# tsilva/gymnasium-solver

Measured on AMD Instinct MI355X. Metric: env steps/sec (rollout+PPO update), CartPole n_envs=4096, 1/2/4/8 MI355X, higher is better.
Workload: dtype f32; 1 GPU; CartPole-v1:ppo C2 (rollout 4096 envs x 32 steps + 20-epoch PPO update, B=256); n_envs_per_gpu=4096, n_steps=32, batch_size=256, n_epochs=20, policy=MLP 4-256-256-{2,1}, parallelism=single, graph=True, same_device=False, dp_mode=local, track_stats=False

## Files before the change

gymnasium-solver_amd/build_lib.py:

```python
from __future__ import annotations

import os
import subprocess
import sys
from concurrent.futures import ThreadPoolExecutor

HERE = os.path.dirname(os.path.abspath(__file__))
CSRC = os.path.join(HERE, "csrc")
BUILD = os.path.join(HERE, "build")
LIB = os.path.join(HERE, "gsamd", "libgsamd.so")
HIPCC = os.environ.get("HIPCC", "/opt/rocm/bin/hipcc")
ARCH = "gfx950"

EXTRA = {"gs_gae.hip": ["-ffp-contract=off"], "gs_mlp.hip": ["-ffp-contract=off"], "gs_atari.hip": ["-ffp-contract=off"],
         "gs_cartpole.hip": ["-ffp-contract=off"]}


def _sources():
    return sorted(f for f in os.listdir(CSRC) if f.endswith((".hip", ".cpp")))


def _obj(src):
    return os.path.join(BUILD, src + ".o")


def _source_hashes(csrc=None):
    sys.path.insert(0, os.path.join(HERE, "gsamd"))
    try:
        import buildinfo
    finally:
# ... 6 lines not shown
def _compile(src, build_dir=None, defines=(), csrc=None, hashes=None):
    csrc = csrc or CSRC
    path = os.path.join(csrc, src)
    obj = os.path.join(build_dir, src + ".o") if build_dir else _obj(src)
    deps = [path, os.path.join(HERE, "..", "include", "gsamd.h")] + [
        os.path.join(csrc, h) for h in os.listdir(csrc) if h.endswith(".h")]
    hdefs = []
    if src == "gs_abi.cpp" and hashes:
        hdefs = [f'-DGS_SRC_HASH_{k}="{v}"' for k, v in sorted(hashes.items())]
        stamp = obj + ".hash"
        if not os.path.exists(stamp) or open(stamp).read() != " ".join(hdefs):
            if os.path.exists(obj):
                os.remove(obj)
            with open(stamp, "w") as f:
                f.write(" ".join(hdefs))
    if os.path.exists(obj) and os.path.getmtime(obj) >= max(os.path.getmtime(d) for d in deps):
        return None
    cmd = [HIPCC, "-O3", "-std=c++17", "-fPIC", "-Wall", "-Wno-unused-function", "-c", path, "-o", obj]
    if src.endswith(".hip"):
        cmd[1:1] = [f"--offload-arch={ARCH}", "-x", "hip"]
    cmd += EXTRA.get(src, []) + [f"-D{d}" for d in defines] + hdefs
    r = subprocess.run(cmd, capture_output=True, text=True)
    if r.returncode != 0:
        raise RuntimeError(f"compile failed: {' '.join(cmd)}\n{r.stdout}\n{r.stderr}")
    return src


def build(verbose: bool = False, jobs: int = 8) -> str:
    os.makedirs(BUILD, exist_ok=True)
    srcs = _sources()
    hashes = _source_hashes()
    with ThreadPoolExecutor(max_workers=min(jobs, len(srcs))) as ex:
        done = [s for s in ex.map(lambda s: _compile(s, hashes=hashes), srcs) if s]
    objs = [_obj(s) for s in srcs]
    if done or not os.path.exists(LIB) or os.path.getmtime(LIB) < max(os.path.getmtime(o) for o in objs):
        cmd = [HIPCC, f"--offload-arch={ARCH}", "-shared", "-fPIC", "-o", LIB] + objs + [
            "-L/opt/rocm/lib", "-lrccl", "-Wl,-rpath,/opt/rocm/lib"]
        r = subprocess.run(cmd, capture_output=True, text=True)
        if r.returncode != 0:
# ... 39 lines not shown
```

gymnasium-solver_amd/csrc/gs_common.h:

```cpp
#pragma once
#include <hip/hip_runtime.h>
#include <stdint.h>
#include <stdio.h>
#include <string>
#include <type_traits>

#include "../../include/gsamd.h"

typedef float f32x4 __attribute__((ext_vector_type(4)));
typedef __bf16 bf16x8 __attribute__((ext_vector_type(8)));

namespace gs {

#ifdef GS_STAMPS
extern __device__ unsigned long long g_stamp_acc[8][16];
extern __device__ unsigned long long g_stamp_cnt[8];
#define GS_STAMP_BEGIN_IF(k, cond)                                                 \
    unsigned long long _st_t[17];                                                  \
    int _st_n = 0;                                                                 \
    const bool _st_on = (cond) && threadIdx.x == 0;                                \
    const int _st_k = (k);                                                         \
    if (_st_on) _st_t[0] = __builtin_amdgcn_s_memtime();
#define GS_STAMP_BEGIN(k) GS_STAMP_BEGIN_IF(k, blockIdx.x == 0 && blockIdx.y == 0)
#define GS_STAMP(i)                                                                \
    if (_st_on) _st_t[(i) + 1] = __builtin_amdgcn_s_memtime();                     \
    _st_n = (i) + 1;
#define GS_STAMP_END(i)                                                            \
    GS_STAMP(i)                                                                    \
    if (_st_on) {                                                                  \
        for (int _j = 0; _j < _st_n; ++_j)                                         \
            atomicAdd(&g_stamp_acc[_st_k][_j], _st_t[_j + 1] - _st_t[_j]);         \
        atomicAdd(&g_stamp_cnt[_st_k], 1ull);                                      \
    }
#else
#define GS_STAMP_BEGIN(k)
#define GS_STAMP_BEGIN_IF(k, cond)
#define GS_STAMP(i)
#define GS_STAMP_END(i)
#endif

void set_error(const char *fmt, ...);
int hip_fail(hipError_t e, const char *what, const char *file, int line);

#define GS_HIP(call)                                                         \
    do {                                                                     \
        hipError_t _e = (call);                                              \
        if (_e != hipSuccess) return gs::hip_fail(_e, #call, __FILE__, __LINE__); \
    } while (0)

#define GS_REQUIRE(cond, ...)                    \
// ... 315 lines not shown
```

gymnasium-solver_amd/csrc/gs_mlp.hip:

```cpp
#include <float.h>

#include <mutex>
#include <unordered_map>

#include "gs_common.h"
#include "gs_xgmi_dev.h"
#include "gs_synth_env.h"

namespace gs {

#ifdef GS_STAMPS
__device__ unsigned long long g_stamp_acc[8][16];
__device__ unsigned long long g_stamp_cnt[8];
#endif
#if defined(GS_STAMPS) || defined(GS_SPANS)
constexpr int kSpanK = 2048, kSpanWG = 288;
__device__ unsigned g_span[2][kSpanK][kSpanWG][9];
__device__ __forceinline__ int span_wg() { return (int)(blockIdx.x + blockIdx.y * gridDim.x); }
__device__ __forceinline__ void span_start(int kern, int64_t k, unsigned long long t0)
{
    if (threadIdx.x == 0 && k >= 0 && k < kSpanK && span_wg() < kSpanWG) g_span[kern][k][span_wg()][0] = (unsigned)t0;
}
__device__ __forceinline__ void span_end(int kern, int64_t k)
{
// ... 168 lines not shown

template <int AMAX, int AEX>
__device__ __forceinline__ void gather_head_row(const float *__restrict__ zpart, const float *__restrict__ P,
                                                const Layout &L, int64_t r, float (&z)[AMAX + 1]);
template <int AMAX>
__device__ __forceinline__ void loss_row(const float (&z)[AMAX + 1], int A, int act, float olp, float ov, float adv,
                                         float ret, const LossArgs &la, float invB, float *__restrict__ dzr,
                                         double (&acc)[14]);

#ifndef GS_FWD_ADAM_NT
#define GS_FWD_ADAM_NT 512
#endif
constexpr int kFwdAdamThreads = GS_FWD_ADAM_NT;
static_assert(kFwdAdamThreads == 256 || kFwdAdamThreads == 512, "lagged forward: 256 or 512 threads");

template <class S, bool FUSED, bool ADAM = false, bool STATS = false>
__global__ __launch_bounds__(ADAM ? kFwdAdamThreads : 256) void k_fwd_hidden(
    const float *__restrict__ P, Layout Lrt, const float *__restrict__ obs, const int32_t *__restrict__ idx, int T,
    int N, int rows, float *__restrict__ x_out, float *__restrict__ h1_out, float *__restrict__ h2_out,
    float *__restrict__ zpart, float *__restrict__ obs_copy, const int32_t *__restrict__ stop, RowGather rg,
    FusedFwd ff, LossArgs la, uint16_t *__restrict__ h2mask, AdamFwd af = AdamFwd{})
{
    GS_STAMP_BEGIN(0)
    GS_SPAN_T0
    if (stop && *stop) return;
    extern __shared__ float lds[];
    const Layout L = S::lay(Lrt);
    const int D = L.D, H1 = L.H1, H2 = L.H2, A1 = L.A + 1;
    const int cb = blockIdx.x, rb = blockIdx.y;
    const int r0 = rb * kTile;
    const int c0 = cb * kTile;
    const int tid = threadIdx.x, lane = tid & 63, wave = tid >> 6;
    constexpr int NT = ADAM ? kFwdAdamThreads : 256;
    const int ldh = H1 + 4;
    int *srcs = reinterpret_cast<int *>(lds);
    float *W1s = lds + 16;
    float *b1s = W1s + round4(H1 * D);
    float *W2s = b1s + round4(H1);
    float *b2s = W2s + kTile * ldh;
    float *whs = b2s + 16;
    float *xs = whs + round4(A1 * 16);
    float *h1s = xs + round4(kTile * D);
    float *red = h1s + kTile * ldh;
    float *h2s = red + 1024;

    if (rg.step_base && idx) idx += *rg.step_base * rows;
    const int64_t kstep = FUSED ? ff.k_local + (ff.step_base ? *ff.step_base : 0) : 0;
    if constexpr (ADAM) GS_SPAN_START(0, kstep)
    constexpr bool kStage0 = FUSED && S::H1c > 0 && (S::H1c * 4) % 4 == 0;
    constexpr int kW2v = S::H1c > 0 ? kTile * S::H1c / 4 / NT : 0;
    float4 w2r[kW2v > 0 ? kW2v : 1];
    static_assert(!ADAM || (kStage0 && kW2v > 0), "lagged Adam: compile-time fused shapes only");
    if constexpr (ADAM) {
        constexpr Layout Lc = S::lay(Layout{});
        constexpr int cD = Lc.D, cH1 = Lc.H1, cA1 = Lc.A + 1, n1 = cH1 * (cD + 1), k4n = cH1 / 4;
        constexpr int NQ = (n1 / 4 + 255) / 256, NRB = (S::Bc + S::RB - 1) / S::RB, NS = 2;
        static_assert(Lc.oW1 == 0 && Lc.oW2 == n1 && (cH1 * cD) % 4 == 0 && cH1 % 4 == 0, "W1|b1: one float4 region");
        static_assert(NRB >= 1 && NRB <= 8 && NQ <= 2 && n1 <= kTile * (cH1 + 4), "lagged-Adam register / LDS budget");
        const AdamArgs &aa = af.aa;
        const bool fold = af.part1 != nullptr;
        const int64_t kprev = kstep - 1 + af.force;
        const bool apply = kprev >= 0;
        const bool own1 = apply && cb == 0 && rb == 0, own2 = apply && rb == 0;
        const bool stW2[3] = {own2, own2, own2};
        const bool stW1[3] = {own1, own1, own1};
        const float4 z4 = make_float4(0.f, 0.f, 0.f, 0.f);
        auto ld4 = [](const float *base, int64_t q) {
            const f32x4 v = *(const __attribute__((address_space(1))) f32x4 *)(base + 4 * q);
            return make_float4(v[0], v[1], v[2], v[3]);
        };
        auto ld1 = [](const float *base, int64_t o) { return *(const __attribute__((address_space(1))) float *)(base + o); };
        constexpr int nq1 = n1 / 4;
        constexpr int NQP = (nq1 + NT - 1) / NT;
        const bool nrm = NT == 256 || tid < 256;
        float sl[NS];
#pragma unroll
        for (int j = 0; j < NS; ++j) sl[j] = ld1(af.sumsq, nrm ? min(tid + 256 * j, aa.n_slots - 1) : 0);
        float4 w1p[NQP], w1m[NQP], w1v[NQP], t[NQ][NRB];
        const float *tsrc = fold ? af.part1 : af.G;
        const int64_t tstride = fold ? (int64_t)n1 : 0;
        const int nrb_used = fold ? NRB : 1;
#pragma unroll
        for (int j = 0; j < NQ; ++j)
#pragma unroll
            for (int b = 0; b < NRB; ++b)
                t[j][b] = ld4(tsrc + (int64_t)b * tstride, nrm ? min(tid + 256 * j, nq1 - 1) : 0);
#pragma unroll
        for (int j = 0; j < NQP; ++j) {
            const int q = min(tid + NT * j, nq1 - 1);
            w1p[j] = ld4(P, q);
            w1m[j] = ld4(af.Min, q);
            w1v[j] = ld4(af.Vin, q);
// ... 433 lines not shown
    }
    const int ncbz = gridDim.x;
    for (int u = tid; u < kTile * A1; u += NT) {
        const int row = u / A1, a = u - row * A1;
        if (r0 + row >= rows) continue;
        float z = 0.0f;
#pragma unroll
        for (int c = 0; c < kTile; ++c) z = fmaf(h2s[row * 17 + c], whs[a * 16 + c], z);
        zpart[((int64_t)(r0 + row) * ncbz + cb) * A1 + a] = z;
    }
    if (!kEarly) store_x_h1(tid, NT);
    GS_STAMP_END(6)
    if constexpr (ADAM) GS_SPAN_END(0, kstep)
}

static int set_lds_limit(const void *fn, size_t bytes);
template <class F>
static int with_shape(const Layout &L, int64_t B, F &&f);

int launch_fwd_hidden(const float *params, const Layout &L, const float *obs, const int32_t *idx, int64_t T,
                      int64_t N, int64_t rows, float *x_out, float *h1_out, float *h2_out, float *zpart,
                      float *obs_copy, const int32_t *stop_flag, const RowGather *rg, hipStream_t s,
                      uint16_t *h2mask)
{
    const dim3 grid((unsigned)((L.H2 + kTile - 1) / kTile), (unsigned)((rows + kTile - 1) / kTile));
    RowGather g{};
    if (rg) g = *rg;
    return with_shape(L, 0, [&](auto sh) {
        using Sh = decltype(sh);
        int rc = set_lds_limit((const void *)k_fwd_hidden<Sh, false>, fwd_lds_bytes(L));
        if (rc) return rc;
        hipLaunchKernelGGL((k_fwd_hidden<Sh, false>), grid, dim3(256), fwd_lds_bytes(L), s, params, L, obs, idx,
                           (int)T, (int)N, (int)rows, x_out, h1_out, h2_out, zpart, obs_copy, stop_flag, g,
                           FusedFwd{}, LossArgs{}, h2_out ? h2mask : (uint16_t *)nullptr);
        GS_LAUNCH_CHECK("k_fwd_hidden");
        return GS_OK;
    });
}

struct HeadRow {
    float lse;
    float m2;
    float S;
};

template <int AMAX>
__device__ __forceinline__ HeadRow head_stats(const float (&z)[AMAX + 1], int A)
{
    float m = -INFINITY;
// ... 660 lines not shown
    }
}

__device__ __forceinline__ void store_metric_groups(const double *dscr, int n, int r0, int B, int64_t k,
                                                    double *__restrict__ mp)
{
    const int ng = n / kTile;
    if ((int)threadIdx.x < ng * kNumSums) {
        const int g = threadIdx.x / kNumSums, q = threadIdx.x - g * kNumSums;
        double t = 0.0;
        for (int i = 0; i < kTile; ++i) t += dscr[(g * kTile + i) * kNumSums + q];
        mp[(k * (B / kTile) + r0 / kTile + g) * kNumSums + q] = t;
    }
}

template <class S, bool FUSED>
__global__ __launch_bounds__(256) void k_bwd(const float *__restrict__ P, Layout Lrt, int Brt,
                                             const float *__restrict__ x, const float *__restrict__ h1,
                                             const float *__restrict__ h2, const float *__restrict__ dz,
                                             float *__restrict__ G, float *__restrict__ part1,
                                             float *__restrict__ sumsq, const int32_t *__restrict__ stop,
                                             const float *__restrict__ zpart, FusedFwd ff, LossArgs la,
                                             const uint16_t *__restrict__ h2mask, BwdXchg bx)
{
    GS_SPAN_T0
    if (stop && *stop) return;
    const bool xchg = bx.world > 1;
    const uint32_t xseq = xchg ? bx.seq[blockIdx.x] + 1u : 0u;
    const int64_t kstep = FUSED ? ff.k_local + (ff.step_base ? *ff.step_base : 0) : 0;
    if constexpr (FUSED) GS_SPAN_START(1, kstep)
    extern __shared__ float lds[];
    __shared__ float sbuf[FUSED ? 3 * 272 : 272];
    const Layout L = S::lay(Lrt);
    const int B = S::batch(Brt);
    const int D = L.D, H1 = L.H1, H2 = L.H2, A = L.A, A1 = A + 1;
    constexpr int kRowsB = S::RB;
    const BwdShape sh = BwdShape::make(L, B, kRowsB);
    const int tid = threadIdx.x, lane = tid & 63, wave = tid >> 6;
    const int li = lane & 15, lq = lane >> 4;
    int bid = (int)blockIdx.x;
    if (bid < sh.nB) bid += sh.nA;
    else if (bid < sh.nB + sh.nA) bid -= sh.nB;

    if (bid < sh.nA) {
// ... 11 lines not shown
        float *red = h1T + kw * ld;
        int *mkA = reinterpret_cast<int *>(red + 3072);
        if constexpr (S::H1c > 0 && S::Bc > 0) {
            constexpr Layout Lc = S::lay(Layout{});
            constexpr int cB = S::Bc, cBp = (cB + 63) / 64 * 64, cncb = (Lc.H2 + kTile - 1) / kTile;
            constexpr int cka = (Lc.H1 / kTile) % 2 == 0 ? 2 : 1, ckw = kTile * cka, cq = ckw / 4;
            constexpr int NMk = (cBp + 255) / 256, NH1 = (cBp * cq + 255) / 256;
            int mr[NMk];
            float4 hr[NH1];
            float wh = 0.0f;
#pragma unroll
            for (int j = 0; j < NMk; ++j) {
                const int b = tid + 256 * j;
                mr[j] = (int)h2mask[(int64_t)min(b, cB - 1) * cncb + nb];
            }
#pragma unroll
            for (int j = 0; j < NH1; ++j) {
                const int u = tid + 256 * j, b = u / cq, c4 = u % cq;
                hr[j] = *reinterpret_cast<const float4 *>(h1 + (int64_t)min(b, cB - 1) * Lc.H1 +
                                                          min(k0 + 4 * c4, Lc.H1 - 4));
            }
            {
                const int a = min(tid >> 4, A1 - 1), j = tid & 15;
                wh = P[L.head_row(a) + min(n0 + j, H2 - 1)];
            }
            if constexpr (FUSED)
                loss_rows_lds<S>(P, L, zpart, ff, la, B, kstep, 0, B, dzs, nullptr);
            else
                copy_to_lds(dzs, dz, B * A1);
            if (tid < A1 * kTile) whs[tid] = n0 + (tid & 15) < H2 ? wh : 0.0f;
// ... 216 lines not shown
            constexpr Layout Lc = S::lay(Layout{});
            constexpr int cH1 = Lc.H1, cH2 = Lc.H2, cD = Lc.D, cA1 = Lc.A + 1, cB = S::Bc;
            constexpr int cncb = (cH2 + kTile - 1) / kTile, cH2p = (cH2 + 63) / 64 * 64;
            constexpr int NM = (kRowsB * cncb + kLd - 1) / kLd, NW = (cH2p * 4 + kLd - 1) / kLd;
            constexpr int NH = (cA1 * cH2 + kLd - 1) / kLd, N1 = (kRowsB * 16 + kLd - 1) / kLd;
            constexpr int NX = (kRowsB * cD + kLd - 1) / kLd;
            if (tid < kLd) {
                int mr[NM];
                float4 wr[NW];
                float hr[NH], h1r[N1], xr[NX];
#pragma unroll
                for (int j = 0; j < NM; ++j) {
                    const int u = min(tid + j * kLd, kRowsB * cncb - 1), i = u / cncb, c = u - i * cncb;
                    mr[j] = (int)h2mask[(int64_t)min(b0 + i, cB - 1) * cncb + c];
                }
#pragma unroll
                for (int j = 0; j < NW; ++j) {
                    const int u = tid + j * kLd, n = min(u >> 2, cH2 - 1), c4 = u & 3;
                    wr[j] = *reinterpret_cast<const float4 *>(P + Lc.oW2 + (int64_t)n * cH1 + min(k0 + 4 * c4, cH1 - 4));
                }
#pragma unroll
                for (int j = 0; j < NH; ++j) {
                    const int u = min(tid + j * kLd, cA1 * cH2 - 1), a = u / cH2, n = u - a * cH2;
                    hr[j] = P[Lc.head_row(a) + n];
                }
#pragma unroll
                for (int j = 0; j < N1; ++j) {
                    const int u = tid + j * kLd, i = min(u >> 4, kRowsB - 1), jj = u & 15;
                    h1r[j] = h1[(int64_t)min(b0 + i, cB - 1) * cH1 + min(k0 + jj, cH1 - 1)];
                }
// ... 54 lines not shown
            }
            for (int u = tid; u < kRowsB * 16; u += kLd) {
                const int i = u >> 4, j = u & 15;
                h1m[u] = (b0 + i < B && k0 + j < H1) ? h1[(int64_t)(b0 + i) * H1 + k0 + j] : 0.0f;
            }
            for (int u = tid; u < kRowsB * D; u += kLd) xs[u] = b0 * D + u < B * D ? x[(int64_t)b0 * D + u] : 0.0f;
        }
#ifdef GS_STAMPS
        const unsigned long long t_rb0 = __builtin_amdgcn_s_memtime();
        if (bid == 0 && tid == 0) {
            asm volatile("s_waitcnt vmcnt(0) lgkmcnt(0)" ::: "memory");
            atomicAdd(&g_stamp_acc[6][0], __builtin_amdgcn_s_memtime() - t_rb0);
            atomicAdd(&g_stamp_cnt[6], 1ull);
        }
#endif
        if constexpr (FUSED)
            loss_rows_lds<S>(P, L, zpart, ff, la, B, kstep, b0, kRowsB, dzs, nullptr, kLd, 256 - kLd);
#ifdef GS_STAMPS
        if (bid == 0 && tid == 192) {
            asm volatile("s_waitcnt vmcnt(0) lgkmcnt(0)" ::: "memory");
            atomicAdd(&g_stamp_acc[7][0], __builtin_amdgcn_s_memtime() - t_rb0);
            atomicAdd(&g_stamp_cnt[7], 1ull);
        }
#endif
        else
            for (int u = tid; u < kRowsB * A1; u += 256)
                dzs[u] = b0 * A1 + u < B * A1 ? dz[(int64_t)b0 * A1 + u] : 0.0f;
        __syncthreads();
        GS_STAMP(0)
        static_assert(kRowsB == 32 || kRowsB == 64, "role-B slabs of 32 or 64 rows");
        const int nchB = H2p / kTile;
        const int rt = kRowsB == 64 ? wave : wave >> 1, half = kRowsB == 64 ? 0 : wave & 1;
        const int chb = half ? nchB / 2 : 0, che = (half || kRowsB == 64) ? nchB : nchB / 2;
        f32x4 acc0 = {0.f, 0.f, 0.f, 0.f}, acc1 = {0.f, 0.f, 0.f, 0.f};
        if (dh2_regs) {
            const int row = rt * 16 + li;
            float dzr[5];
#pragma unroll
            for (int a = 0; a < 5; ++a) dzr[a] = a < A1 ? dzs[row * A1 + a] : 0.0f;
            const float *brow = W2T + li * ld;
            auto dh2_cols = [&](int ch, float (&av)[4]) {
                const int n = ch * kTile + 4 * lq;
// ... 209 lines not shown
                loss_rows_lds<S>(P, L, zpart, ff, la, B, kstep, 0, Bp, dzs, ge > gs ? dscrC : nullptr, 0, 256,
                                 kTile * gs, kTile * ge);
            else
                for (int u = tid; u < Bp * A1; u += 256) dzs[u] = u < B * A1 ? dz[u] : 0.0f;
        };
        if constexpr (S::H1c > 0 && S::Bc > 0) {
            constexpr Layout Lc = S::lay(Layout{});
            constexpr int cB = S::Bc, cBp = (cB + 15) / 16 * 16, NH = (cBp * 4 + 255) / 256;
            float4 hr[NH];
#pragma unroll
            for (int j = 0; j < NH; ++j) {
                const int u = tid + 256 * j, b = u >> 2, c4 = u & 3;
                hr[j] = *reinterpret_cast<const float4 *>(h2 + (int64_t)min(b, cB - 1) * Lc.H2 +
                                                          min(n0 + 4 * c4, Lc.H2 - 4));
            }
            loss_in();
#pragma unroll
            for (int j = 0; j < NH; ++j) {
                const int u = tid + 256 * j, b = u >> 2, c4 = u & 3;
                if (u < cBp * 4) {
                    const bool ok = b < cB && n0 + 4 * c4 < Lc.H2;
                    hs[b * 17 + 4 * c4 + 0] = ok ? hr[j].x : 0.0f;
                    hs[b * 17 + 4 * c4 + 1] = ok ? hr[j].y : 0.0f;
                    hs[b * 17 + 4 * c4 + 2] = ok ? hr[j].z : 0.0f;
                    hs[b * 17 + 4 * c4 + 3] = ok ? hr[j].w : 0.0f;
                }
            }
        } else {
#pragma unroll 4
            for (int u = tid; u < Bp * 4; u += 256) {
// ... 117 lines not shown
            bool ok[1] = {tid < A1};
            if (tid < A1)
#pragma unroll
                for (int m = 0; m < 16; ++m) bv[0] += partC[tid * 16 + m];
            if (xchg) bwd_exchange<1>(bx, xseq, bv, ok);
            if (ok[0]) {
                G[L.head_bias(tid)] = bv[0];
                sqb = bv[0] * bv[0];
            }
            block_sumsq_store(sqb, sumsq + sh.nT + 2 * sh.ncb, sbuf);
            if constexpr (FUSED) store_head_split(sbuf, A, ff.headsq, (kstep * (sh.ncb + 1) + sh.ncb) * 2);
        }
        GS_STAMP_END(1)
        if constexpr (FUSED) GS_SPAN_END(1, kstep)
    }
}


template <class S, int NRB, int NQ>
__global__ __launch_bounds__(256) void k_clip_adam(float *__restrict__ Pm, Layout Lrt, float *__restrict__ G,
                                                   float *__restrict__ M, float *__restrict__ V,
                                                   const float *__restrict__ part1, const float *__restrict__ sumsq,
                                                   AdamArgs aa, float *__restrict__ metrics,
                                                   const int32_t *__restrict__ stop)
{
    if (stop && *stop) {
        if (metrics && blockIdx.x == 0 && threadIdx.x == 0) {
            float *m = metrics + (aa.step_base ? *aa.step_base : 0) * GS_NUM_METRICS;
            m[GS_M_SKIPPED] = 1.0f;
            m[GS_M_KL_STOP] = 1.0f;
// ... 232 lines not shown

static int set_lds_limit(const void *fn, size_t bytes)
{
    static std::mutex mu;
    static std::unordered_map<const void *, size_t> done;
    if (bytes <= 65536) return GS_OK;
    std::lock_guard<std::mutex> lk(mu);
    auto it = done.find(fn);
    if (it != done.end() && it->second >= bytes) return GS_OK;
    GS_HIP(hipFuncSetAttribute(fn, hipFuncAttributeMaxDynamicSharedMemorySize, (int)bytes));
    done[fn] = bytes;
    return GS_OK;
}

template <class Sh>
constexpr bool bf16_shape()
{
    if constexpr (Sh::AEX == 0 || Sh::H1c == 0 || Sh::Bc == 0) {
        return false;
    } else {
        constexpr Layout Lc = Sh::lay(Layout{});
        return Lc.A + 1 <= 5 && Lc.H2 % 64 == 0;
    }
}

bool has_bf16_chain(const Layout &L, int64_t B)
{
    bool ok = false;
    with_shape(L, B, [&](auto sh) {
        ok = bf16_shape<decltype(sh)>();
// ... 7 lines not shown
    if (has_bf16_chain(L, B)) {
        const int rc = with_shape(L, B, [&](auto sh) {
            using Sh = decltype(sh);
            if constexpr (bf16_shape<Sh>())
                return set_lds_limit((const void *)k_bwd<Bf16Shape<Sh>, true>, bwd_lds_bytes(L, B));
            return GS_OK;
        });
        if (rc) return rc;
    }
    int rc = with_shape(L, B, [&](auto sh) {
        return set_lds_limit((const void *)k_bwd<decltype(sh), false>, bwd_lds_bytes(L, B));
    });
    if (rc) return rc;
    if (has_fused(L, B)) {
        rc = with_shape(L, B, [&](auto sh) {
            return set_lds_limit((const void *)k_bwd<decltype(sh), true>, bwd_lds_bytes(L, B));
        });
        if (rc) return rc;
    }
    rc = with_shape(L, 0, [&](auto sh) {
        return set_lds_limit((const void *)k_fwd_hidden<decltype(sh), false>, fwd_lds_bytes(L));
    });
    if (rc) return rc;
    if (!has_fused(L, B)) return GS_OK;
    return with_shape(L, B, [&](auto sh) {
        return set_lds_limit((const void *)k_fwd_hidden<decltype(sh), true>, fwd_lds_bytes(L));
    });
}

int launch_heads_act(const float *P, const Layout &L, const float *zpart, int64_t rows, int mode, uint64_t seed,
                     uint64_t counter, int64_t *actions, float *logp, float *value, hipStream_t s,
                     const uint64_t *clock)
{
    const dim3 grid((unsigned)((rows + 255) / 256));
    return with_shape(L, 0, [&](auto sh) {
        hipLaunchKernelGGL(k_heads_act<decltype(sh)>, grid, dim3(256), 0, s, P, L, zpart, rows, mode, seed, counter,
                           actions, logp, value, clock);
        GS_LAUNCH_CHECK("k_heads_act");
        return GS_OK;
    });
}

// ... 30 lines not shown
    return (int64_t)(colocated - 1) * nblk < (int64_t)ncu * per_cu;
}

int launch_bwd(const float *P, const Layout &L, int64_t B, const Workspace &ws, float *G, const int32_t *stop,
               hipStream_t s, const FusedFwd *ff, const LossArgs *la, const BwdXchg *bxp)
{
    const BwdShape sh0 = BwdShape::make(L, (int)B, rows_b(L, B));
    const unsigned nblk = (unsigned)(sh0.nA + sh0.nB + sh0.nC);
    const size_t lds = bwd_lds_bytes(L, B);
    BwdXchg bx{};
    if (bxp && bxp->world > 1) {
        GS_REQUIRE(bwd_xchg_fits(L, B), "k_bwd exchange: %u workgroups or their output slots exceed the limits",
                   nblk);
        bx = *bxp;
    }
    return with_shape(L, B, [&](auto sh) {
        using Sh = decltype(sh);
        if (ff && la && la->bf16) {
            if constexpr (bf16_shape<Sh>()) {
                int rc = set_lds_limit((const void *)k_bwd<Bf16Shape<Sh>, true>, lds);
                if (rc) return rc;
                hipLaunchKernelGGL((k_bwd<Bf16Shape<Sh>, true>), dim3(nblk), dim3(256), lds, s, P, L, (int)B, ws.x,
                                   ws.h1, ws.h2, ws.dz, G, ws.part1, ws.sumsq, stop, ws.zpart, *ff, *la, ws.h2mask, bx);
                GS_LAUNCH_CHECK("k_bwd<bf16>");
                return GS_OK;
            } else {
                GS_REQUIRE(false, "precision bf16: no bf16 instantiation of the MLP chain for this shape");
            }
        }
        if (ff) {
            int rc = set_lds_limit((const void *)k_bwd<Sh, true>, lds);
            if (rc) return rc;
            hipLaunchKernelGGL((k_bwd<Sh, true>), dim3(nblk), dim3(256), lds, s, P, L, (int)B, ws.x, ws.h1, ws.h2,
                               ws.dz, G, ws.part1, ws.sumsq, stop, ws.zpart, *ff, *la, ws.h2mask, bx);
        } else {
            int rc = set_lds_limit((const void *)k_bwd<Sh, false>, lds);
            if (rc) return rc;
            hipLaunchKernelGGL((k_bwd<Sh, false>), dim3(nblk), dim3(256), lds, s, P, L, (int)B, ws.x, ws.h1, ws.h2,
                               ws.dz, G, ws.part1, ws.sumsq, stop, (const float *)nullptr, FusedFwd{}, LossArgs{},
                               ws.h2mask, bx);
        }
        GS_LAUNCH_CHECK("k_bwd");
// ... 466 lines not shown
bool has_lagged(const Layout &L, int64_t B)
{
    bool ok = false;
    with_shape(L, B, [&](auto sh) {
        ok = lagged_shape<decltype(sh)>() && n_sumsq_slots(L) <= 512;
        return GS_OK;
    });
    return ok && has_fused(L, B);
}

int launch_fwd_fused(const float *params, const Layout &L, int64_t B, const FusedFwd &ff, const LossArgs &la,
                     const Workspace &ws, const int32_t *stop, hipStream_t s, const AdamFwd *af)
{
    const dim3 grid((unsigned)((L.H2 + kTile - 1) / kTile), (unsigned)((B + kTile - 1) / kTile));
    GS_REQUIRE(!ff.act || (L.D <= 8 && L.H1 <= L.H2), "activation statistics in the fused forward: D <= 8, H1 <= H2");
    return with_shape(L, B, [&](auto sh) {
        using Sh = decltype(sh);
        auto go = [&](auto stats) -> int {
            constexpr bool ST = decltype(stats)::value && (Sh::H1c > 0);
            const float *no_obs = nullptr;
            const int32_t *no_idx = nullptr;
            float *no_copy = nullptr;
            if (la.bf16) {
                if constexpr (bf16_shape<Sh>() && lagged_shape<Sh>()) {
                    using Sb = Bf16Shape<Sh>;
                    if (af) {
                        GS_REQUIRE((af->part1 ? af->aa.nrb > 0 : af->aa.nrb == 0) && af->aa.n_slots <= 512,
                                   "lagged Adam: bad slot / partial counts");
                        hipLaunchKernelGGL((k_fwd_hidden<Sb, true, true, ST>), grid, dim3(kFwdAdamThreads),
                                           fwd_lds_bytes(L), s, params, L, no_obs, no_idx, 0, 0, (int)B, ws.x, ws.h1,
                                           ws.h2, ws.zpart, no_copy, stop, RowGather{}, ff, la, ws.h2mask, *af);
                    } else {
                        hipLaunchKernelGGL((k_fwd_hidden<Sb, true, false, ST>), grid, dim3(256), fwd_lds_bytes(L), s,
                                           params, L, no_obs, no_idx, 0, 0, (int)B, ws.x, ws.h1, ws.h2, ws.zpart,
                                           no_copy, stop, RowGather{}, ff, la, ws.h2mask, AdamFwd{});
                    }
                    GS_LAUNCH_CHECK("k_fwd_hidden<fused, bf16>");
                    return GS_OK;
                } else {
                    GS_REQUIRE(false, "precision bf16: no bf16 instantiation of the MLP chain for this shape");
                }
            }
            if (af) {
                if constexpr (lagged_shape<Sh>()) {
                    GS_REQUIRE((af->part1 ? af->aa.nrb > 0 : af->aa.nrb == 0) && af->aa.n_slots <= 512,
                               "lagged Adam: bad slot / partial counts");
                    hipLaunchKernelGGL((k_fwd_hidden<Sh, true, true, ST>), grid, dim3(kFwdAdamThreads),
                                       fwd_lds_bytes(L), s, params, L, no_obs, no_idx, 0, 0, (int)B, ws.x, ws.h1,
                                       ws.h2, ws.zpart, no_copy, stop, RowGather{}, ff, la, ws.h2mask, *af);
                    GS_LAUNCH_CHECK("k_fwd_hidden<fused, adam>");
                    return GS_OK;
                } else {
                    GS_REQUIRE(false, "lagged Adam: no compile-time instantiation for this shape");
                }
            }
            hipLaunchKernelGGL((k_fwd_hidden<Sh, true, false, ST>), grid, dim3(256), fwd_lds_bytes(L), s, params, L,
                               no_obs, no_idx, 0, 0, (int)B, ws.x, ws.h1, ws.h2, ws.zpart, no_copy, stop, RowGather{},
                               ff, la, ws.h2mask, AdamFwd{});
            GS_LAUNCH_CHECK("k_fwd_hidden<fused>");
            return GS_OK;
        };
        return ff.act ? go(std::true_type{}) : go(std::false_type{});
    });
}

__global__ __launch_bounds__(256) void k_act_stats_fused(const uint32_t *__restrict__ act, int nrb, int ncb, int H1,
                                                         int H2, int B, float *__restrict__ metrics)
{
    __shared__ double sred[4 * (256 + 16)];
    __shared__ unsigned smax[2];
    const int64_t k = blockIdx.x;
    const int tid = threadIdx.x;
    const uint32_t *a = act + k * (int64_t)nrb * ncb * kActRec;
    if (tid < 2) smax[tid] = 0u;
    __syncthreads();
    double dsum[2] = {0.0, 0.0};
#pragma unroll
// ... 110 lines not shown
```

Before: 885,100 env_steps/s.

## Add lean chain kernel entries with preloaded kernargs for fused PPO forward/backward

Splits the fused forward and backward kernels into device bodies with new slim __global__ entries (k_fwd_chain, k_bwd_chain). The entries take a small argument list plus a packed tail struct, drop the stop-flag and step-base loads at compile time when they are unused, and skip the cross-device exchange path. It also enables AMDGPU kernarg preloading for the first 14 arguments and forces recompiles when compile flags change. The aim is to cut kernel-entry latency (kernarg loads and scalar setup) in the many small graph-launched PPO update kernels, at the cost of more template instantiations and host-side checks that the field arrays share one stride.

```diff
diff --git a/gymnasium-solver_amd/build_lib.py b/gymnasium-solver_amd/build_lib.py
--- a/gymnasium-solver_amd/build_lib.py
+++ b/gymnasium-solver_amd/build_lib.py
@@ -14,6 +14,9 @@
 
 EXTRA = {"gs_gae.hip": ["-ffp-contract=off"], "gs_mlp.hip": ["-ffp-contract=off"], "gs_atari.hip": ["-ffp-contract=off"],
          "gs_cartpole.hip": ["-ffp-contract=off"]}
+KERNARG_PRELOAD = os.environ.get("GSAMD_KERNARG_PRELOAD", "1") != "0"
+if KERNARG_PRELOAD:
+    EXTRA["gs_mlp.hip"] = EXTRA["gs_mlp.hip"] + ["-mllvm", "-amdgpu-kernarg-preload-count=14"]
 
 
 def _sources():
@@ -50,15 +53,21 @@
                 os.remove(obj)
             with open(stamp, "w") as f:
                 f.write(" ".join(hdefs))
-    if os.path.exists(obj) and os.path.getmtime(obj) >= max(os.path.getmtime(d) for d in deps):
-        return None
     cmd = [HIPCC, "-O3", "-std=c++17", "-fPIC", "-Wall", "-Wno-unused-function", "-c", path, "-o", obj]
     if src.endswith(".hip"):
         cmd[1:1] = [f"--offload-arch={ARCH}", "-x", "hip"]
     cmd += EXTRA.get(src, []) + [f"-D{d}" for d in defines] + hdefs
+    flags = obj + ".flags"
+    want = " ".join(EXTRA.get(src, []))
+    if os.path.exists(obj) and (not os.path.exists(flags) or open(flags).read() != want):
+        os.remove(obj)
+    if os.path.exists(obj) and os.path.getmtime(obj) >= max(os.path.getmtime(d) for d in deps):
+        return None
     r = subprocess.run(cmd, capture_output=True, text=True)
     if r.returncode != 0:
         raise RuntimeError(f"compile failed: {' '.join(cmd)}\n{r.stdout}\n{r.stderr}")
+    with open(flags, "w") as f:
+        f.write(want)
     return src
 
 
diff --git a/gymnasium-solver_amd/csrc/gs_common.h b/gymnasium-solver_amd/csrc/gs_common.h
--- a/gymnasium-solver_amd/csrc/gs_common.h
+++ b/gymnasium-solver_amd/csrc/gs_common.h
@@ -18,6 +18,7 @@
 #define GS_STAMP_BEGIN_IF(k, cond)                                                 \
     unsigned long long _st_t[17];                                                  \
     int _st_n = 0;                                                                 \
+    unsigned long long _st_entry = 0;                                              \
     const bool _st_on = (cond) && threadIdx.x == 0;                                \
     const int _st_k = (k);                                                         \
     if (_st_on) _st_t[0] = __builtin_amdgcn_s_memtime();
@@ -25,15 +26,21 @@
 #define GS_STAMP(i)                                                                \
     if (_st_on) _st_t[(i) + 1] = __builtin_amdgcn_s_memtime();                     \
     _st_n = (i) + 1;
+#define GS_STAMP_T0 const unsigned long long _st_t0 = __builtin_amdgcn_s_memtime();
+#define GS_STAMP_ENTRY                                                             \
+    if (_st_on) _st_entry = __builtin_amdgcn_s_memtime() - _st_t0;
 #define GS_STAMP_END(i)                                                            \
     GS_STAMP(i)                                                                    \
     if (_st_on) {                                                                  \
+        atomicAdd(&g_stamp_acc[_st_k][15], _st_entry);                             \
         for (int _j = 0; _j < _st_n; ++_j)                                         \
             atomicAdd(&g_stamp_acc[_st_k][_j], _st_t[_j + 1] - _st_t[_j]);         \
         atomicAdd(&g_stamp_cnt[_st_k], 1ull);                                      \
     }
 #else
 #define GS_STAMP_BEGIN(k)
+#define GS_STAMP_T0
+#define GS_STAMP_ENTRY
 #define GS_STAMP_BEGIN_IF(k, cond)
 #define GS_STAMP(i)
 #define GS_STAMP_END(i)
diff --git a/gymnasium-solver_amd/csrc/gs_mlp.hip b/gymnasium-solver_amd/csrc/gs_mlp.hip
--- a/gymnasium-solver_amd/csrc/gs_mlp.hip
+++ b/gymnasium-solver_amd/csrc/gs_mlp.hip
@@ -206,16 +206,18 @@
 constexpr int kFwdAdamThreads = GS_FWD_ADAM_NT;
 static_assert(kFwdAdamThreads == 256 || kFwdAdamThreads == 512, "lagged forward: 256 or 512 threads");
 
-template <class S, bool FUSED, bool ADAM = false, bool STATS = false>
-__global__ __launch_bounds__(ADAM ? kFwdAdamThreads : 256) void k_fwd_hidden(
-    const float *__restrict__ P, Layout Lrt, const float *__restrict__ obs, const int32_t *__restrict__ idx, int T,
-    int N, int rows, float *__restrict__ x_out, float *__restrict__ h1_out, float *__restrict__ h2_out,
-    float *__restrict__ zpart, float *__restrict__ obs_copy, const int32_t *__restrict__ stop, RowGather rg,
-    FusedFwd ff, LossArgs la, uint16_t *__restrict__ h2mask, AdamFwd af = AdamFwd{})
+template <class S, bool FUSED, bool ADAM, bool STATS, bool BASE>
+__device__ __forceinline__ void fwd_hidden_body(
+    const float *__restrict__ P, const Layout &Lrt, const float *__restrict__ obs, const int32_t *__restrict__ idx,
+    int T, int N, int rows, float *__restrict__ x_out, float *__restrict__ h1_out, float *__restrict__ h2_out,
+    float *__restrict__ zpart, float *__restrict__ obs_copy, const int32_t *__restrict__ stop, const RowGather &rg,
+    const FusedFwd &ff, uint16_t *__restrict__ h2mask, const AdamFwd &af)
 {
     GS_STAMP_BEGIN(0)
     GS_SPAN_T0
-    if (stop && *stop) return;
+    GS_STAMP_T0
+    if constexpr (!FUSED)
+        if (stop && *stop) return;
     extern __shared__ float lds[];
     const Layout L = S::lay(Lrt);
     const int D = L.D, H1 = L.H1, H2 = L.H2, A1 = L.A + 1;
@@ -236,8 +238,10 @@
     float *red = h1s + kTile * ldh;
     float *h2s = red + 1024;
 
-    if (rg.step_base && idx) idx += *rg.step_base * rows;
-    const int64_t kstep = FUSED ? ff.k_local + (ff.step_base ? *ff.step_base : 0) : 0;
+    if constexpr (!FUSED)
+        if (rg.step_base && idx) idx += *rg.step_base * rows;
+    int64_t kstep = FUSED ? ff.k_local : 0;
+    if constexpr (FUSED && BASE) kstep += ff.step_base ? *ff.step_base : 0;
     if constexpr (ADAM) GS_SPAN_START(0, kstep)
     constexpr bool kStage0 = FUSED && S::H1c > 0 && (S::H1c * 4) % 4 == 0;
     constexpr int kW2v = S::H1c > 0 ? kTile * S::H1c / 4 / NT : 0;
@@ -268,6 +272,7 @@
         float sl[NS];
 #pragma unroll
         for (int j = 0; j < NS; ++j) sl[j] = ld1(af.sumsq, nrm ? min(tid + 256 * j, aa.n_slots - 1) : 0);
+        GS_STAMP_ENTRY
         float4 w1p[NQP], w1m[NQP], w1v[NQP], t[NQ][NRB];
         const float *tsrc = fold ? af.part1 : af.G;
         const int64_t tstride = fold ? (int64_t)n1 : 0;
@@ -731,6 +736,53 @@
     if constexpr (ADAM) GS_SPAN_END(0, kstep)
 }
 
+template <class S, bool FUSED>
+__global__ __launch_bounds__(256) void k_fwd_hidden(
+    const float *__restrict__ P, Layout Lrt, const float *__restrict__ obs, const int32_t *__restrict__ idx, int T,
+    int N, int rows, float *__restrict__ x_out, float *__restrict__ h1_out, float *__restrict__ h2_out,
+    float *__restrict__ zpart, float *__restrict__ obs_copy, const int32_t *__restrict__ stop, RowGather rg,
+    uint16_t *__restrict__ h2mask)
+{
+    static_assert(!FUSED, "the fused chain's forward enters through k_fwd_chain");
+    fwd_hidden_body<S, false, false, false, false>(P, Lrt, obs, idx, T, N, rows, x_out, h1_out, h2_out, zpart,
+                                                   obs_copy, stop, rg, FusedFwd{}, h2mask, AdamFwd{});
+}
+
+struct FwdTail {
+    const float *xg;
+    const int64_t *step_base;
+    float *x_out, *h1_out, *h2_out, *zpart;
+    uint16_t *h2mask;
+    float *Pout, *Mout, *Vout;
+    float *metrics;
+    double *normsq;
+    const float *sched;
+    uint32_t *act;
+    float max_norm, one_minus_b1, b2, one_minus_b2, neg_step_size, inv_bc2_sqrt, eps, grad_scale;
+    int force;
+};
+template <class S, bool ADAM, bool STATS, bool BASE>
+__global__ __launch_bounds__(ADAM ? kFwdAdamThreads : 256) void k_fwd_chain(
+    const float *__restrict__ sumsq, const float *__restrict__ part1, const float *__restrict__ P,
+    const float *__restrict__ Min, const float *__restrict__ Vin, const float *__restrict__ G, int n_slots,
+    int k_local, FwdTail t)
+{
+    static_assert(S::Bc > 0 && S::H1c > 0, "chain entry: compile-time shapes only");
+    FusedFwd ff{};
+    ff.xg = t.xg, ff.step_base = t.step_base, ff.k_local = k_local, ff.act = t.act;
+    AdamFwd af{};
+    if constexpr (ADAM) {
+        af.Min = Min, af.Vin = Vin, af.G = G, af.part1 = part1, af.sumsq = sumsq;
+        af.Pout = t.Pout, af.Mout = t.Mout, af.Vout = t.Vout, af.metrics = t.metrics, af.force = t.force;
+        af.aa.max_norm = t.max_norm, af.aa.one_minus_b1 = t.one_minus_b1, af.aa.b2 = t.b2;
+        af.aa.one_minus_b2 = t.one_minus_b2, af.aa.neg_step_size = t.neg_step_size;
+        af.aa.inv_bc2_sqrt = t.inv_bc2_sqrt, af.aa.eps = t.eps, af.aa.grad_scale = t.grad_scale;
+        af.aa.n_slots = n_slots, af.aa.sched = t.sched, af.aa.normsq = t.normsq;
+    }
+    fwd_hidden_body<S, true, ADAM, STATS, BASE>(P, Layout{}, nullptr, nullptr, 0, 0, S::Bc, t.x_out, t.h1_out, t.h2_out,
+                                                t.zpart, nullptr, nullptr, RowGather{}, ff, t.h2mask, af);
+}
+
 static int set_lds_limit(const void *fn, size_t bytes);
 template <class F>
 static int with_shape(const Layout &L, int64_t B, F &&f);
@@ -749,7 +801,7 @@
         if (rc) return rc;
         hipLaunchKernelGGL((k_fwd_hidden<Sh, false>), grid, dim3(256), fwd_lds_bytes(L), s, params, L, obs, idx,
                            (int)T, (int)N, (int)rows, x_out, h1_out, h2_out, zpart, obs_copy, stop_flag, g,
-                           FusedFwd{}, LossArgs{}, h2_out ? h2mask : (uint16_t *)nullptr);
+                           h2_out ? h2mask : (uint16_t *)nullptr);
         GS_LAUNCH_CHECK("k_fwd_hidden");
         return GS_OK;
     });
@@ -1440,20 +1492,23 @@
     }
 }
 
-template <class S, bool FUSED>
-__global__ __launch_bounds__(256) void k_bwd(const float *__restrict__ P, Layout Lrt, int Brt,
-                                             const float *__restrict__ x, const float *__restrict__ h1,
-                                             const float *__restrict__ h2, const float *__restrict__ dz,
-                                             float *__restrict__ G, float *__restrict__ part1,
-                                             float *__restrict__ sumsq, const int32_t *__restrict__ stop,
-                                             const float *__restrict__ zpart, FusedFwd ff, LossArgs la,
-                                             const uint16_t *__restrict__ h2mask, BwdXchg bx)
+template <class S, bool FUSED, bool XCHG, bool BASE>
+__device__ __forceinline__ void bwd_body(const float *__restrict__ P, const Layout &Lrt, int Brt,
+                                         const float *__restrict__ x, const float *__restrict__ h1,
+                                         const float *__restrict__ h2, const float *__restrict__ dz,
+                                         float *__restrict__ G, float *__restrict__ part1,
+                                         float *__restrict__ sumsq, const int32_t *__restrict__ stop,
+                                         const float *__restrict__ zpart, const FusedFwd &ff, const LossArgs &la,
+                                         const uint16_t *__restrict__ h2mask, const BwdXchg &bx)
 {
     GS_SPAN_T0
-    if (stop && *stop) return;
-    const bool xchg = bx.world > 1;
+    GS_STAMP_T0
+    if constexpr (!FUSED)
+        if (stop && *stop) return;
+    const bool xchg = XCHG && bx.world > 1;
     const uint32_t xseq = xchg ? bx.seq[blockIdx.x] + 1u : 0u;
-    const int64_t kstep = FUSED ? ff.k_local + (ff.step_base ? *ff.step_base : 0) : 0;
+    int64_t kstep = FUSED ? ff.k_local : 0;
+    if constexpr (FUSED && BASE) kstep += ff.step_base ? *ff.step_base : 0;
     if constexpr (FUSED) GS_SPAN_START(1, kstep)
     extern __shared__ float lds[];
     __shared__ float sbuf[FUSED ? 3 * 272 : 272];
@@ -1495,6 +1550,7 @@
                 const int b = tid + 256 * j;
                 mr[j] = (int)h2mask[(int64_t)min(b, cB - 1) * cncb + nb];
             }
+            GS_STAMP_ENTRY
 #pragma unroll
             for (int j = 0; j < NH1; ++j) {
                 const int u = tid + 256 * j, b = u / cq, c4 = u % cq;
@@ -1741,6 +1797,7 @@
                     const int u = min(tid + j * kLd, kRowsB * cncb - 1), i = u / cncb, c = u - i * cncb;
                     mr[j] = (int)h2mask[(int64_t)min(b0 + i, cB - 1) * cncb + c];
                 }
+                GS_STAMP_ENTRY
 #pragma unroll
                 for (int j = 0; j < NW; ++j) {
                     const int u = tid + j * kLd, n = min(u >> 2, cH2 - 1), c4 = u & 3;
@@ -1825,8 +1882,12 @@
             atomicAdd(&g_stamp_cnt[6], 1ull);
         }
 #endif
-        if constexpr (FUSED)
+        if constexpr (FUSED) {
             loss_rows_lds<S>(P, L, zpart, ff, la, B, kstep, b0, kRowsB, dzs, nullptr, kLd, 256 - kLd);
+        } else {
+            for (int u = tid; u < kRowsB * A1; u += 256)
+                dzs[u] = b0 * A1 + u < B * A1 ? dz[(int64_t)b0 * A1 + u] : 0.0f;
+        }
 #ifdef GS_STAMPS
         if (bid == 0 && tid == 192) {
             asm volatile("s_waitcnt vmcnt(0) lgkmcnt(0)" ::: "memory");
@@ -1834,9 +1895,6 @@
             atomicAdd(&g_stamp_cnt[7], 1ull);
         }
 #endif
-        else
-            for (int u = tid; u < kRowsB * A1; u += 256)
-                dzs[u] = b0 * A1 + u < B * A1 ? dz[(int64_t)b0 * A1 + u] : 0.0f;
         __syncthreads();
         GS_STAMP(0)
         static_assert(kRowsB == 32 || kRowsB == 64, "role-B slabs of 32 or 64 rows");
@@ -2076,6 +2134,7 @@
                 hr[j] = *reinterpret_cast<const float4 *>(h2 + (int64_t)min(b, cB - 1) * Lc.H2 +
                                                           min(n0 + 4 * c4, Lc.H2 - 4));
             }
+            GS_STAMP_ENTRY
             loss_in();
 #pragma unroll
             for (int j = 0; j < NH; ++j) {
@@ -2223,6 +2282,42 @@
         GS_STAMP_END(1)
         if constexpr (FUSED) GS_SPAN_END(1, kstep)
     }
+}
+
+template <class S, bool FUSED>
+__global__ __launch_bounds__(256) void k_bwd(const float *__restrict__ P, Layout Lrt, int Brt,
+                                             const float *__restrict__ x, const float *__restrict__ h1,
+                                             const float *__restrict__ h2, const float *__restrict__ dz,
+                                             float *__restrict__ G, float *__restrict__ part1,
+                                             float *__restrict__ sumsq, const int32_t *__restrict__ stop,
+                                             const float *__restrict__ zpart, FusedFwd ff, LossArgs la,
+                                             const uint16_t *__restrict__ h2mask, BwdXchg bx)
+{
+    bwd_body<S, FUSED, true, true>(P, Lrt, Brt, x, h1, h2, dz, G, part1, sumsq, stop, zpart, ff, la, h2mask, bx);
+}
+
+struct BwdTail {
+    const float *h2;
+    float *G, *part1, *sumsq;
+    double *mpart;
+    float *headsq;
+    const int64_t *step_base;
+    LossArgs la;
+};
+template <class S, bool BASE>
+__global__ __launch_bounds__(256) void k_bwd_chain(const float *__restrict__ P, const float *__restrict__ h1,
+                                                   const uint16_t *__restrict__ h2mask,
+                                                   const float *__restrict__ zpart, const float *__restrict__ fields,
+                                                   const float *__restrict__ x, int fstride, int k_local, BwdTail t)
+{
+    static_assert(S::Bc > 0 && S::H1c > 0, "chain entry: compile-time shapes only");
+    FusedFwd ff{};
+    ff.fa = reinterpret_cast<const int32_t *>(fields);
+    ff.folp = fields + fstride, ff.fov = fields + 2 * (int64_t)fstride;
+    ff.fadv = fields + 3 * (int64_t)fstride, ff.fret = fields + 4 * (int64_t)fstride;
+    ff.mpart = t.mpart, ff.headsq = t.headsq, ff.step_base = t.step_base, ff.k_local = k_local;
+    bwd_body<S, true, false, BASE>(P, Layout{}, S::Bc, x, h1, t.h2, nullptr, t.G, t.part1, t.sumsq, nullptr, zpart, ff,
+                                   t.la, h2mask, BwdXchg{});
 }
 
 
@@ -2485,6 +2580,9 @@
 }
 
 template <class Sh>
+constexpr bool chain_shape() { return Sh::AEX > 0 && Sh::H1c > 0 && Sh::Bc > 0; }
+
+template <class Sh>
 constexpr bool bf16_shape()
 {
     if constexpr (Sh::AEX == 0 || Sh::H1c == 0 || Sh::Bc == 0) {
@@ -2522,7 +2620,18 @@
     if (rc) return rc;
     if (has_fused(L, B)) {
         rc = with_shape(L, B, [&](auto sh) {
-            return set_lds_limit((const void *)k_bwd<decltype(sh), true>, bwd_lds_bytes(L, B));
+            using Sh = decltype(sh);
+            const size_t lds = bwd_lds_bytes(L, B);
+            int r = set_lds_limit((const void *)k_bwd<Sh, true>, lds);
+            if constexpr (chain_shape<Sh>()) {
+                if (!r) r = set_lds_limit((const void *)k_bwd_chain<Sh, false>, lds);
+                if (!r) r = set_lds_limit((const void *)k_bwd_chain<Sh, true>, lds);
+                if constexpr (bf16_shape<Sh>()) {
+                    if (!r) r = set_lds_limit((const void *)k_bwd_chain<Bf16Shape<Sh>, false>, lds);
+                    if (!r) r = set_lds_limit((const void *)k_bwd_chain<Bf16Shape<Sh>, true>, lds);
+                }
+            }
+            return r;
         });
         if (rc) return rc;
     }
@@ -2531,9 +2640,8 @@
     });
     if (rc) return rc;
     if (!has_fused(L, B)) return GS_OK;
-    return with_shape(L, B, [&](auto sh) {
-        return set_lds_limit((const void *)k_fwd_hidden<decltype(sh), true>, fwd_lds_bytes(L));
-    });
+    GS_REQUIRE(fwd_lds_bytes(L) <= 65536, "fused forward: %zu bytes of LDS exceed the default limit", fwd_lds_bytes(L));
+    return GS_OK;
 }
 
 int launch_heads_act(const float *P, const Layout &L, const float *zpart, int64_t rows, int mode, uint64_t seed,
@@ -2594,10 +2702,39 @@
                    nblk);
         bx = *bxp;
     }
+    GS_REQUIRE(!ff || !stop, "the fused chain takes no stop flag (it runs only without a KL early stop)");
+    GS_REQUIRE(!ff || la, "fused backward: no loss arguments");
+    const bool lean = ff && bx.world <= 1;
+    BwdTail t{};
+    int64_t fstride = 0;
+    if (lean) {
+        fstride = ff->folp - reinterpret_cast<const float *>(ff->fa);
+        GS_REQUIRE(fstride > 0 && fstride < ((int64_t)1 << 29) && ff->fov == ff->folp + fstride &&
+                       ff->fadv == ff->fov + fstride && ff->fret == ff->fadv + fstride,
+                   "fused backward: the per-update field arrays are not at one stride");
+        t.h2 = ws.h2, t.G = G, t.part1 = ws.part1, t.sumsq = ws.sumsq;
+        t.mpart = ff->mpart, t.headsq = ff->headsq, t.step_base = ff->step_base, t.la = *la;
+    }
     return with_shape(L, B, [&](auto sh) {
         using Sh = decltype(sh);
-        if (ff && la && la->bf16) {
+        auto chain = [&](auto shape) -> int {
+            using S = decltype(shape);
+            const float *fields = reinterpret_cast<const float *>(ff->fa);
+            const void *fn = ff->step_base ? (const void *)k_bwd_chain<S, true> : (const void *)k_bwd_chain<S, false>;
+            int rc = set_lds_limit(fn, lds);
+            if (rc) return rc;
+            if (ff->step_base)
+                hipLaunchKernelGGL((k_bwd_chain<S, true>), dim3(nblk), dim3(256), lds, s, P, ws.h1, ws.h2mask, ws.zpart,
+                                   fields, ws.x, (int)fstride, ff->k_local, t);
+            else
+                hipLaunchKernelGGL((k_bwd_chain<S, false>), dim3(nblk), dim3(256), lds, s, P, ws.h1, ws.h2mask,
+                                   ws.zpart, fields, ws.x, (int)fstride, ff->k_local, t);
+            GS_LAUNCH_CHECK("k_bwd_chain");
+            return GS_OK;
+        };
+        if (ff && la->bf16) {
             if constexpr (bf16_shape<Sh>()) {
+                if (lean) return chain(Bf16Shape<Sh>{});
                 int rc = set_lds_limit((const void *)k_bwd<Bf16Shape<Sh>, true>, lds);
                 if (rc) return rc;
                 hipLaunchKernelGGL((k_bwd<Bf16Shape<Sh>, true>), dim3(nblk), dim3(256), lds, s, P, L, (int)B, ws.x,
@@ -2606,6 +2743,13 @@
                 return GS_OK;
             } else {
                 GS_REQUIRE(false, "precision bf16: no bf16 instantiation of the MLP chain for this shape");
+            }
+        }
+        if (lean) {
+            if constexpr (chain_shape<Sh>()) {
+                return chain(sh);
+            } else {
+                GS_REQUIRE(false, "fused backward: no compile-time instantiation for this shape");
             }
         }
         if (ff) {
@@ -3102,53 +3246,59 @@
 {
     const dim3 grid((unsigned)((L.H2 + kTile - 1) / kTile), (unsigned)((B + kTile - 1) / kTile));
     GS_REQUIRE(!ff.act || (L.D <= 8 && L.H1 <= L.H2), "activation statistics in the fused forward: D <= 8, H1 <= H2");
+    GS_REQUIRE(!stop, "the fused chain takes no stop flag (it runs only without a KL early stop)");
+    GS_REQUIRE(!af || ((af->part1 ? af->aa.nrb > 0 : af->aa.nrb == 0) && af->aa.n_slots <= 512),
+               "lagged Adam: bad slot / partial counts");
+    FwdTail t{};
+    t.xg = ff.xg, t.step_base = ff.step_base, t.act = ff.act;
+    t.x_out = ws.x, t.h1_out = ws.h1, t.h2_out = ws.h2, t.zpart = ws.zpart, t.h2mask = ws.h2mask;
+    const AdamFwd a = af ? *af : AdamFwd{};
+    t.Pout = a.Pout, t.Mout = a.Mout, t.Vout = a.Vout, t.metrics = a.metrics, t.normsq = a.aa.normsq;
+    t.sched = a.aa.sched, t.force = a.force;
+    t.max_norm = a.aa.max_norm, t.one_minus_b1 = a.aa.one_minus_b1, t.b2 = a.aa.b2, t.one_minus_b2 = a.aa.one_minus_b2;
+    t.neg_step_size = a.aa.neg_step_size, t.inv_bc2_sqrt = a.aa.inv_bc2_sqrt, t.eps = a.aa.eps;
+    t.grad_scale = a.aa.grad_scale;
+    const int k_local = ff.k_local;
     return with_shape(L, B, [&](auto sh) {
         using Sh = decltype(sh);
-        auto go = [&](auto stats) -> int {
-            constexpr bool ST = decltype(stats)::value && (Sh::H1c > 0);
-            const float *no_obs = nullptr;
-            const int32_t *no_idx = nullptr;
-            float *no_copy = nullptr;
+        if constexpr (!chain_shape<Sh>()) {
+            GS_REQUIRE(false, "fused forward: no compile-time instantiation for this shape");
+        } else {
+            auto go = [&](auto shape, auto stats, auto base) -> int {
+                using S = decltype(shape);
+                constexpr bool ST = decltype(stats)::value, BS = decltype(base)::value;
+                if (af) {
+                    if constexpr (lagged_shape<Sh>()) {
+                        hipLaunchKernelGGL((k_fwd_chain<S, true, ST, BS>), grid, dim3(kFwdAdamThreads),
+                                           fwd_lds_bytes(L), s, a.sumsq, a.part1, params, a.Min, a.Vin, a.G,
+                                           a.aa.n_slots, k_local, t);
+                        GS_LAUNCH_CHECK("k_fwd_chain<adam>");
+                        return GS_OK;
+                    } else {
+                        GS_REQUIRE(false, "lagged Adam: no compile-time instantiation for this shape");
+                    }
+                }
+                const float *none = nullptr;
+                hipLaunchKernelGGL((k_fwd_chain<S, false, ST, BS>), grid, dim3(256), fwd_lds_bytes(L), s, none, none,
+                                   params, none, none, none, 0, k_local, t);
+                GS_LAUNCH_CHECK("k_fwd_chain");
+                return GS_OK;
+            };
+            auto go_sb = [&](auto shape) -> int {
+                if (ff.act) return ff.step_base ? go(shape, std::true_type{}, std::true_type{})
+                                                : go(shape, std::true_type{}, std::false_type{});
+                return ff.step_base ? go(shape, std::false_type{}, std::true_type{})
+                                    : go(shape, std::false_type{}, std::false_type{});
+            };
             if (la.bf16) {
                 if constexpr (bf16_shape<Sh>() && lagged_shape<Sh>()) {
-                    using Sb = Bf16Shape<Sh>;
-                    if (af) {
-                        GS_REQUIRE((af->part1 ? af->aa.nrb > 0 : af->aa.nrb == 0) && af->aa.n_slots <= 512,
-                                   "lagged Adam: bad slot / partial counts");
-                        hipLaunchKernelGGL((k_fwd_hidden<Sb, true, true, ST>), grid, dim3(kFwdAdamThreads),
-                                           fwd_lds_bytes(L), s, params, L, no_obs, no_idx, 0, 0, (int)B, ws.x, ws.h1,
-                                           ws.h2, ws.zpart, no_copy, stop, RowGather{}, ff, la, ws.h2mask, *af);
-                    } else {
-                        hipLaunchKernelGGL((k_fwd_hidden<Sb, true, false, ST>), grid, dim3(256), fwd_lds_bytes(L), s,
-                                           params, L, no_obs, no_idx, 0, 0, (int)B, ws.x, ws.h1, ws.h2, ws.zpart,
-                                           no_copy, stop, RowGather{}, ff, la, ws.h2mask, AdamFwd{});
-                    }
-                    GS_LAUNCH_CHECK("k_fwd_hidden<fused, bf16>");
-                    return GS_OK;
+                    return go_sb(Bf16Shape<Sh>{});
                 } else {
                     GS_REQUIRE(false, "precision bf16: no bf16 instantiation of the MLP chain for this shape");
                 }
             }
-            if (af) {
-                if constexpr (lagged_shape<Sh>()) {
-                    GS_REQUIRE((af->part1 ? af->aa.nrb > 0 : af->aa.nrb == 0) && af->aa.n_slots <= 512,
-                               "lagged Adam: bad slot / partial counts");
-                    hipLaunchKernelGGL((k_fwd_hidden<Sh, true, true, ST>), grid, dim3(kFwdAdamThreads),
-                                       fwd_lds_bytes(L), s, params, L, no_obs, no_idx, 0, 0, (int)B, ws.x, ws.h1,
-                                       ws.h2, ws.zpart, no_copy, stop, RowGather{}, ff, la, ws.h2mask, *af);
-                    GS_LAUNCH_CHECK("k_fwd_hidden<fused, adam>");
-                    return GS_OK;
-                } else {
-                    GS_REQUIRE(false, "lagged Adam: no compile-time instantiation for this shape");
-                }
-            }
-            hipLaunchKernelGGL((k_fwd_hidden<Sh, true, false, ST>), grid, dim3(256), fwd_lds_bytes(L), s, params, L,
-                               no_obs, no_idx, 0, 0, (int)B, ws.x, ws.h1, ws.h2, ws.zpart, no_copy, stop, RowGather{},
-                               ff, la, ws.h2mask, AdamFwd{});
-            GS_LAUNCH_CHECK("k_fwd_hidden<fused>");
-            return GS_OK;
-        };
-        return ff.act ? go(std::true_type{}) : go(std::false_type{});
+            return go_sb(sh);
+        }
     });
 }
 
```

Result: faster. 956,500 env_steps/s (median of 6 runs) (+8.1%).
